# MinJunKang/DualPixelFace

Measured on AMD Instinct MI355X. Metric: train samples/sec, StereoDPNet 1024x1536 DP pair, higher is better.
Workload: dtype f32

## Files before the change

dualpixelface_amd/csrc/conv_igemm2.hip:

```cpp
#include "conv_internal.h"
#include <cstdlib>
#include <type_traits>

namespace {

constexpr int MAXT = 27;
constexpr int NLD = 8;
constexpr int ZPAGE = 16;

struct G2P {
  int N, C, K, Ktot, k0;
  int ID, IH, IW, OD, OH, OW;
  int sxd, sxh, sxw;
  int e0d, e0h, e0w;
  int ext_d, ext_h;
  int pz, thp, thp_shift, odt;
  int planeStride;
  int RS, SR;
  int colshift;
  int rpc, chanStride;
  int nseg;
  int nwseg;
  int T;
  int tilesH, tilesW;
// ... 914 lines not shown
    } else {
      wpk[base] = (unsigned short)(sh & 0xffffu);
      wpk[base + 512LL * MT] = (unsigned short)(sm & 0xffffu);
      wpk[base + 1024LL * MT] = (unsigned short)(sl & 0xffffu);
    }
  }
}

struct T2P {
  int N, C, K, Ktot, k0;
  int ID, IH, IW, OD, OH, OW;
  int RS, SR, rpc, chanStride, nseg, nwseg, nchunks;
  int tilesH, tilesW, ntiles, cpx, QD;
  unsigned mSR, mRPC, mEH;
  int vec;
};

struct T2Combo { int cls, tap; };
struct T2Unit { int e, n; T2Combo c[8]; };
struct T2Table { T2Unit u[8]; };

constexpr T2Table t2_table() {
  T2Table tb{};
  const int order[8] = {0, 1, 2, 3, 5, 6, 7, 4};
  for (int ui = 0; ui < 8; ++ui) {
    const int e = order[ui];
    const int es[3] = {e >> 2, (e >> 1) & 1, e & 1};
    T2Unit& u = tb.u[ui];
    u.e = e;
    u.n = 0;
// ... 200 lines not shown
      const int od = 2 * qd + rd, oh = 2 * qh + rh, ow = 2 * qw;
      if (od >= p.OD || oh >= p.OH || ow >= p.OW) continue;
      float* op = on + ((long long)od * p.OH + oh) * p.OW + ow;
      if (quad_ok) {
        const bool odd = (l31 & 1) != 0;
#pragma unroll
        for (int j = 0; j < 16; j += 2) {
          const float a0 = acc[rd * 4 + rh * 2][j], a1 = acc[rd * 4 + rh * 2 + 1][j];
          const float b0 = acc[rd * 4 + rh * 2][j + 1], b1 = acc[rd * 4 + rh * 2 + 1][j + 1];
          const float s0 = odd ? a0 : b0, s1 = odd ? a1 : b1;
          const float t0 = __builtin_bit_cast(float, __builtin_amdgcn_mov_dpp(__builtin_bit_cast(int, s0), 0xB1, 0xf, 0xf, true));
          const float t1 = __builtin_bit_cast(float, __builtin_amdgcn_mov_dpp(__builtin_bit_cast(int, s1), 0xB1, 0xf, 0xf, true));
          const int k = ((j + (odd ? 1 : 0)) & 3) + 8 * (j >> 2) + 4 * hh;
          if (k < p.K) {
            const float bv = bias ? bias[p.k0 + k] : 0.f;
            const f32x4 v = odd ? f32x4{t0 + bv, t1 + bv, b0 + bv, b1 + bv} : f32x4{a0 + bv, a1 + bv, t0 + bv, t1 + bv};
            *reinterpret_cast<f32x4*>(on + ((long long)od * p.OH + oh) * p.OW + (ow & ~3) + (long long)k * kstride) = v;
          }
        }
        continue;
      }
#pragma unroll
      for (int j = 0; j < 16; ++j) {
        const int k = (j & 3) + 8 * (j >> 2) + 4 * hh;
        if (k < p.K) {
          const float bv = bias ? bias[p.k0 + k] : 0.f;
          const float v0 = acc[rd * 4 + rh * 2][j] + bv, v1 = acc[rd * 4 + rh * 2 + 1][j] + bv;
          float* o = op + (long long)k * kstride;
          if (pair_ok) {
            *reinterpret_cast<float2*>(o) = make_float2(v0, v1);
          } else {
            o[0] = v0;
            if (ow + 1 < p.OW) o[1] = v1;
          }
        }
      }
    }
}

__global__ void igemm2_pack_kernel(const float* __restrict__ w, float* __restrict__ wpk, int wA, int wB, int T, int KT, int CC, int nchunks,
                                   int mode, int k0, int K, int C) {
  const long long total = (long long)nchunks * T * CC * KT + ZPAGE;
  for (long long i = (long long)blockIdx.x * blockDim.x + threadIdx.x; i < total; i += (long long)gridDim.x * blockDim.x) {
    float v = 0.f;
    if (i >= ZPAGE) {
      const long long e = i - ZPAGE;
      const int k = (int)(e % KT);
      const int cc = (int)((e / KT) % CC);
// ... 184 lines not shown
  p.N = d.N; p.C = d.C; p.Ktot = d.Ktot;
  p.ID = d.ID; p.IH = d.IH; p.IW = d.IW; p.OD = d.OD; p.OH = d.OH; p.OW = d.OW;
  p.RS = 36; p.SR = 9; p.rpc = 2 * 5; p.chanStride = p.rpc * p.RS;
  p.nseg = CC * p.rpc * p.SR;
  p.nwseg = bf ? 27 * 32 : 27 * CC * 32 / 4;
  p.nchunks = (d.C + CC - 1) / CC;
  p.QD = dpf_div_up(d.OD, 2);
  p.tilesH = dpf_div_up(dpf_div_up(d.OH, 2), 4);
  p.tilesW = dpf_div_up(dpf_div_up(d.OW, 2), 32);
  const long long ntiles = (long long)d.N * p.QD * p.tilesH * p.tilesW;
  if (ntiles <= 0 || ntiles > 0x3fffffffLL) return DPF_ERR_INVALID_ARG;
  p.ntiles = (int)ntiles;
  p.cpx = (int)((ntiles + 7) / 8);
  p.mSR = magic20(p.SR); p.mRPC = magic20(p.rpc); p.mEH = magic20(5);
  p.vec = env_int("DPF_G2_VEC_STORE", 1);
  const size_t lds = 2 * (size_t)(CC * p.chanStride + 4 * p.nwseg) * sizeof(float);
  for (int k0 = 0; k0 < d.K; k0 += 32) {
    const int Kc = d.K - k0 < 32 ? d.K - k0 : 32;
    p.K = Kc; p.k0 = d.k0 + k0;
    const long long total = (long long)p.nchunks * 27 * CC * 32 + ZPAGE;
    if (bf)
      hipLaunchKernelGGL(igemm2_pack_bf16_kernel, dim3(dpf_ew_grid(total)), dim3(256), 0, st, w, reinterpret_cast<unsigned short*>(ws), d.wA, d.wB, 27,
                         32, p.nchunks, d.mode, p.k0, Kc, d.C);
    else
      hipLaunchKernelGGL(igemm2_pack_kernel, dim3(dpf_ew_grid(total)), dim3(256), 0, st, w, ws, d.wA, d.wB, 27, 32, CC, p.nchunks, d.mode, p.k0, Kc, d.C);
    if (dpf_check_launch() != DPF_OK) return DPF_ERR_LAUNCH;
    int rc;
    if (bf) {
      rc = launch_t2<8, true>(x, ws, bias, out, p, lds, st);
      if (rc != DPF_OK) return rc;
// ... 14 lines not shown
  const long long x9 = (g4 > g8 ? g4 : g8) * 3 * (KT / 32) * 256;
  return plain > x9 ? plain : x9;
}

int dpf_igemm2_conv(const float* x, const float* w, const float* bias, float* out, float* ws, const DpfConvDesc& d, hipStream_t st,
                    DpfConvStats* stats) {
  static const int enabled = env_int("DPF_IGEMM2", 1);
  if (!enabled) return DPF_ERR_UNSUPPORTED;
  const int T = d.kd * d.kh * d.kw;
  if (T > MAXT || d.K > 128) return DPF_ERR_UNSUPPORTED;
  if ((d.IW & 3) || (reinterpret_cast<uintptr_t>(x) & 15) || (reinterpret_cast<uintptr_t>(ws) & 15)) return DPF_ERR_UNSUPPORTED;
  const long long x_chan = (long long)d.ID * d.IH * d.IW;
  if (9 * x_chan >= (1LL << 30)) return DPF_ERR_UNSUPPORTED;
  if (T == 1 && !env_int("DPF_IGEMM2_1x1", 1)) return DPF_ERR_UNSUPPORTED;
  if (stats && (d.transposed || d.Ktot != d.K)) return DPF_ERR_UNSUPPORTED;
  if (d.accumulate && d.transposed && (d.sd != 1 || d.sh != 1 || d.sw != 1)) return DPF_ERR_UNSUPPORTED;
  if (d.transposed && (d.sd != 1 || d.sh != 1 || d.sw != 1)) return igemm2_tr2(x, w, bias, out, ws, d, st);

  const int MT = (d.K + 31) / 32, KT = 32 * MT;
  static const int nt_over = 0, cc_over = 0, lds_target = 53 * 1024;
  int NT = MT == 1 ? 4 : 2;
  if (nt_over == 2 || (nt_over == 4 && MT <= 2)) NT = nt_over;
  bool bf = dpf_conv_operand_bf16() != 0 && T > 1;
  const bool bf_mode = bf;
  static const int bf3_on = env_int("DPF_IGEMM3_BF", 1);
  int p_single = 0;
  if (bf) {
    auto patch_for = [&](int nt) {
      const int sxh = d.transposed ? 1 : d.sh, sxw = d.transposed ? 1 : d.sw;
      const int e0w = d.transposed ? d.pw - (d.kw - 1) * d.dw : -d.pw;
      const int ext_d = (d.kd - 1) * d.dd + 1, ext_h = (4 * nt - 1) * sxh + (d.kh - 1) * d.dh + 1, ext_w = 31 * sxw + (d.kw - 1) * d.dw + 1;
// ... 184 lines not shown
```

dualpixelface_amd/csrc/norm_act.hip:

```cpp
#include "dpf_common.h"

namespace {

constexpr int ROW_CHUNK = 4096;

template <bool DET> struct RedAcc { typedef float type; };
template <> struct RedAcc<true> { typedef double type; };

__device__ __forceinline__ float red_block_sum(float v, float* sm4) { return dpf_block_sum_256(v, sm4); }
__device__ __forceinline__ float red_block_sum(double v, float* sm4) {
#pragma unroll
  for (int o = 32; o > 0; o >>= 1) v += __shfl_xor(v, o, 64);
  double* smd = reinterpret_cast<double*>(sm4);
  const int w = threadIdx.x >> 6;
  __syncthreads();
  if ((threadIdx.x & 63) == 0) smd[w] = v;
  __syncthreads();
  return (float)((smd[0] + smd[1]) + (smd[2] + smd[3]));
}

template <bool DET>
__global__ __launch_bounds__(256) void bn_stats_kernel(const float* __restrict__ x, float* __restrict__ sums, int N, int C, long long S,
                                                       int chunk) {
  __shared__ float sm[8];
// ... 273 lines not shown
  if (ACT == DPF_ACT_PRELU) {
    const float slf = red_block_sum(sl, sm);
    if (threadIdx.x == 0) atomicAdd(&sums[3 * c + 2], slf);
  }
}

template <int ACT, bool RES>
__global__ __launch_bounds__(256) void bn_bwd_apply_kernel(const float* __restrict__ x, const float* __restrict__ dy,
                                                           const float* __restrict__ mean, const float* __restrict__ invstd,
                                                           const float* __restrict__ w, const float* __restrict__ bsh, int wmod,
                                                           const float* __restrict__ res, int act, const float* __restrict__ slope_p,
                                                           float slope_c, const float* __restrict__ sums, float inv_count,
                                                           int training, float* __restrict__ dx, float* __restrict__ dres, int C,
                                                           long long S, const float* __restrict__ count_dev, int gC = 0, int gc0 = 0,
                                                           float* __restrict__ fin_dweight = nullptr, float* __restrict__ fin_dbias = nullptr,
                                                           float* __restrict__ fin_dslope = nullptr) {
  const int row = blockIdx.y;
  if (blockIdx.x == 0 && blockIdx.y == 0 && (fin_dweight || fin_dbias || fin_dslope)) {
    for (int cp = threadIdx.x; cp < wmod; cp += 256) {
      float a = 0.f, b = 0.f;
      for (int c = cp; c < C; c += wmod) {
        a += sums[3 * c];
        b += sums[3 * c + 1];
      }
      if (fin_dbias) fin_dbias[cp] = a;
      if (fin_dweight) fin_dweight[cp] = b;
    }
    if (fin_dslope && threadIdx.x == 0) {
      float sl = 0.f;
      for (int c = 0; c < C; ++c) sl += sums[3 * c + 2];
      fin_dslope[0] = sl;
// ... 23 lines not shown
    const float z = fmaf(xh, g, be) + rv;
    o_dz = d * dact_t<ACT>(z, slope);
    o_dx = mean ? gi * (o_dz - m_dz - xh * m_dzx) : o_dz;
  };
  (void)act;
  if ((S & 3) == 0) {
#pragma unroll 2
    for (long long s = s0 + 4 * threadIdx.x; s < s1; s += 4 * 256) {
      const v4f xv = ld4(x + base + s);
      const v4f dv = ld4(dy + base + s);
      v4f rv = {0.f, 0.f, 0.f, 0.f};
      if (RES) rv = ld4(res + base + s);
      float z0, z1, z2, z3, x0, x1, x2, x3;
      one(xv.x, rv.x, dv.x, z0, x0); one(xv.y, rv.y, dv.y, z1, x1);
      one(xv.z, rv.z, dv.z, z2, x2); one(xv.w, rv.w, dv.w, z3, x3);
      if (dres) *reinterpret_cast<v4f*>(dres + base + s) = v4f{z0, z1, z2, z3};
      if (dx) *reinterpret_cast<v4f*>(dx + base + s) = v4f{x0, x1, x2, x3};
    }
  } else {
    for (long long s = s0 + threadIdx.x; s < s1; s += 256) {
      float oz, ox;
      one(x[base + s], RES ? res[base + s] : 0.f, dy[base + s], oz, ox);
      if (dres) dres[base + s] = oz;
      if (dx) dx[base + s] = ox;
    }
  }
}

__global__ void bn_bwd_finalize_kernel(const float* __restrict__ sums, int C, int wmod, float* __restrict__ dweight,
                                       float* __restrict__ dbias, float* __restrict__ dslope) {
  const int cp = blockIdx.x * blockDim.x + threadIdx.x;
  if (cp < wmod) {
    float a = 0.f, b = 0.f;
    for (int c = cp; c < C; c += wmod) {
      a += sums[3 * c];
      b += sums[3 * c + 1];
    }
    if (dbias) dbias[cp] = a;
    if (dweight) dweight[cp] = b;
// ... 117 lines not shown
int dpf_norm_act_forward_slice(const float* x, const float* mean, const float* invstd, const float* w, const float* b, int wmod,
                               const float* res, const float* res2, int act, const float* slope, float slope_const, float* y, int y_channels,
                               int y_c0, int N, int C, long long S, void* stream) {
  dpf_clear_error();
  if (!x || !y || N <= 0 || C <= 0 || S <= 0 || (long long)N * C > 65535 || y_c0 < 0 || y_c0 + C > y_channels) return DPF_ERR_INVALID_ARG;
  if (wmod <= 0) wmod = C;
#define DPF_CALL(A, R) hipLaunchKernelGGL((bn_apply_kernel<A, R>), row_grid(N * C, S), dim3(256), 0, (hipStream_t)stream, x, mean, invstd, w, b, wmod, res, res2, act, slope, slope_const, y, C, S, y_channels, y_c0)
  DPF_ACT_DISPATCH(act, (res != nullptr || res2 != nullptr), DPF_CALL)
#undef DPF_CALL
  return dpf_check_launch();
}

static int norm_act_backward_impl(const float* x, const float* dy, int gC, int gc0, const float* mean, const float* invstd, const float* w,
                                  const float* b, int wmod, const float* res, int act, const float* slope, float slope_const, int training,
                                  float* dx, float* dres, float* dweight, float* dbias, float* dslope, float* ws, int N, int C, long long S,
                                  int phase, double count, void* stream) {
  dpf_clear_error();
  if (!x || !dy || !ws || N <= 0 || C <= 0 || S <= 0 || (long long)N * C > 65535 || phase < 0 || phase > 3) return DPF_ERR_INVALID_ARG;
  if (wmod <= 0) wmod = C;
  hipStream_t st = (hipStream_t)stream;
  const bool need_reduce = (mean != nullptr) || (act == DPF_ACT_PRELU && dslope);
  bool fused_fin = false;
  if (need_reduce && phase != 2) {
    if (phase != 3 && hipMemsetAsync(ws, 0, sizeof(float) * 3 * C, st) != hipSuccess) return DPF_ERR_LAUNCH;
    const int chunk = reduce_chunk(N * C, S);
    const bool det = dpf_deterministic() != 0;
#define DPF_CALL(A, R)                                                                                                                              \
  do {                                                                                                                                              \
    if (det) hipLaunchKernelGGL((bn_bwd_reduce_kernel<A, R, true>), dim3(1, (unsigned)C), dim3(256), 0, st, x, dy, mean, invstd, w, b, wmod, res, \
                                act, slope, slope_const, ws, N, C, S, chunk, gC, gc0);                                                             \
    else hipLaunchKernelGGL((bn_bwd_reduce_kernel<A, R, false>), reduce_grid(N * C, S, chunk), dim3(256), 0, st, x, dy, mean, invstd, w, b, wmod,   \
// ... 1 lines not shown
  } while (0)
    DPF_ACT_DISPATCH(act, (res != nullptr), DPF_CALL)
#undef DPF_CALL
    fused_fin = (dx || dres) && phase != 1;
    if (!fused_fin)
      hipLaunchKernelGGL(bn_bwd_finalize_kernel, dim3(dpf_div_up(wmod, 64)), dim3(64), 0, st, ws, C, wmod, mean ? dweight : nullptr,
                         mean ? dbias : nullptr, act == DPF_ACT_PRELU ? dslope : nullptr);
  }
  if ((dx || dres) && phase != 1) {
    const float* count_dev = (phase == 2 && count < 0) ? ws + 3 * (long long)C : nullptr;
    if (count <= 0) count = (double)N * (double)S;
    const float inv_cnt = (float)(1.0 / count);
    float* fdw = (fused_fin && mean) ? dweight : nullptr;
    float* fdb = (fused_fin && mean) ? dbias : nullptr;
    float* fds = (fused_fin && act == DPF_ACT_PRELU) ? dslope : nullptr;
#define DPF_CALL(A, R) hipLaunchKernelGGL((bn_bwd_apply_kernel<A, R>), row_grid(N * C, S), dim3(256), 0, st, x, dy, mean, invstd, w, b, wmod, res, act, slope, slope_const, ws, inv_cnt, training, dx, dres, C, S, count_dev, gC, gc0, fdw, fdb, fds)
    DPF_ACT_DISPATCH(act, (res != nullptr), DPF_CALL)
#undef DPF_CALL
  }
  return dpf_check_launch();
}

int dpf_norm_act_backward_ex(const float* x, const float* dy, const float* mean, const float* invstd, const float* w, const float* b,
                             int wmod, const float* res, int act, const float* slope, float slope_const, int training, float* dx,
                             float* dres, float* dweight, float* dbias, float* dslope, float* ws, int N, int C, long long S, int phase,
                             double count, void* stream) {
  return norm_act_backward_impl(x, dy, 0, 0, mean, invstd, w, b, wmod, res, act, slope, slope_const, training, dx, dres, dweight, dbias,
                                dslope, ws, N, C, S, phase, count, stream);
}

int dpf_norm_act_backward_slice(const float* x, const float* dy, int dy_channels, int dy_c0, const float* mean, const float* invstd,
                                const float* w, const float* b, int wmod, const float* res, int act, const float* slope, float slope_const,
                                int training, float* dx, float* dres, float* dweight, float* dbias, float* dslope, float* ws, int N, int C,
                                long long S, void* stream) {
  if (dy_c0 < 0 || dy_c0 + C > dy_channels) return DPF_ERR_INVALID_ARG;
  return norm_act_backward_impl(x, dy, dy_channels, dy_c0, mean, invstd, w, b, wmod, res, act, slope, slope_const, training, dx, dres,
                                dweight, dbias, dslope, ws, N, C, S, 0, 0.0, stream);
}

int dpf_norm_act_backward_slice_ex(const float* x, const float* dy, int dy_channels, int dy_c0, const float* mean, const float* invstd,
                                   const float* w, const float* b, int wmod, const float* res, int act, const float* slope, float slope_const,
                                   int training, float* dx, float* dres, float* dweight, float* dbias, float* dslope, float* ws, int N, int C,
                                   long long S, int phase, double count, void* stream) {
// ... 23 lines not shown
```

dualpixelface_amd/ops.py:

```python
import ctypes
import os

import torch

from ._lib import lib, DpfError, ERRORS

ACT_NONE, ACT_RELU, ACT_PRELU, ACT_LEAKY, ACT_SIGMOID = 0, 1, 2, 3, 4
BN_EPS, BN_MOMENTUM = 1e-5, 0.1
FUSE_BN_STATS = os.environ.get('DPF_FUSE_BN_STATS', '1') != '0'

_scratch = {}

PROFILE = None
PROFILE_DETAIL = False


class _Timed(object):
    def __init__(self, family, flops, tag='', nbytes=0.0):
        self.family, self.flops, self.tag, self.nbytes = family, flops, tag, nbytes

    def __enter__(self):
        if PROFILE is not None:
            self.e0 = torch.cuda.Event(enable_timing=True)
            self.e1 = torch.cuda.Event(enable_timing=True)
# ... 186 lines not shown
    ws = _conv_ws((kd, kh, kw), C, K, x.device)
    with _dense_timed('fwd', x, K, (kd, kh, kw), stride, dil, od * oh * ow, x.numel() + out.numel() + w.numel()):
        if stats is not None and FUSE_BN_STATS and K <= 128 and IW % 4 == 0 and kd * kh * kw > 1:
            cap = int(L.call('dpf_conv_stats_slab_doubles', N, K, od, oh, ow))
            slab = torch.empty(cap, dtype=torch.float64, device=x.device)
            parts = ctypes.c_int(0)
            if _supported('dpf_conv_forward_stats', _ptr(x), _ptr(w), _ptr(bias), _ptr(out), _ptr(ws), N, C, ID, IH, IW, K, kd, kh, kw,
                          *stride, *pad, *dil, _ptr(slab), cap, ctypes.byref(parts), _stream()):
                stats.update(slab=slab, parts=int(parts.value), count=N * od * oh * ow, channels=K, ptr=out.data_ptr())
                return out
        L.call('dpf_conv_forward', _ptr(x), _ptr(w), _ptr(bias), _ptr(out), _ptr(ws), N, C, ID, IH, IW, K, kd, kh, kw,
               *stride, *pad, *dil, _stream())
    return out


def _conv_transpose_raw(x, w, bias, out_dims, ksize, stride, pad, dil, k_needed=None):
    N, C, ID, IH, IW = x.shape
    K = w.shape[1]
    kd, kh, kw = ksize
    out = torch.empty((N, K) + tuple(out_dims), dtype=torch.float32, device=x.device)
    L = lib()
    if (C <= 4 and bias is None and k_needed is None and tuple(stride) == (1, 1, 1) and tuple(dil) == (1, 1, 1) and kh == 3 and kw == 3
            and out_dims[2] % 4 == 0):
        with _Timed('conv_smallk', 2.0 * N * K * C * kd * kh * kw * ID * IH * IW, 'skd N%d C%d K%d in%dx%dx%d' % (N, C, K, ID, IH, IW)):
            done = _supported('dpf_conv_smallk_dgrad', _ptr(x), _ptr(w), _ptr(out), N, K, *out_dims, C, kd, kh, kw, *pad, _stream())
        if done:
            return out
    if k_needed is not None and 0 < k_needed < K:
        out[:, k_needed:].zero_()
        entry, chans = 'dpf_conv_transpose_ex', (k_needed, K)
    else:
        entry, chans = 'dpf_conv_transpose', (K,)
    ws = _conv_ws(ksize, C, K, x.device)
    with _dense_timed('tr ', x, chans[0], ksize, stride, dil, ID * IH * IW, x.numel() + out.numel() * chans[0] // K + w.numel()):
        L.call(entry, _ptr(x), _ptr(w), _ptr(bias), _ptr(out), _ptr(ws), N, C, ID, IH, IW, *chans, *out_dims, kd, kh, kw,
# ... 76 lines not shown
        gw = _conv_wgrad_raw(g, x, wshape, stride, pad, dil)
    g.record_stream(side)
    x.record_stream(side)
    _wgrad_pending.append((p, gw.view(p.shape)))
    return None


def _channel_sum(g):
    N, C = g.shape[0], g.shape[1]
    S = g.numel() // (N * C)
    out = torch.zeros(C, dtype=torch.float32, device=g.device)
    lib().call('dpf_channel_sum', _ptr(g), _ptr(out), N, C, S, _stream())
    return out


class ConvFn(torch.autograd.Function):

    @staticmethod
    def forward(ctx, x, w, bias, stride, pad, dil, gi_channels=None, stats=None):
        x, w = _c(x), _c(w)
        _need(x, w, bias)
        ctx.cfg = (stride, pad, dil)
        ctx.gi_channels = gi_channels
        ctx.save_for_backward(x, w)
        ctx.has_bias = bias is not None
        ctx.bf16 = CONV_OPERANDS_BF16
        return _conv_fwd_raw(x, w, bias, stride, pad, dil, stats)

    @staticmethod
    def backward(ctx, gy):
        x, w = ctx.saved_tensors
        stride, pad, dil = ctx.cfg
        gy = _c(gy)
        gx = gw = gb = None
        with conv_operands(ctx.bf16):
            if ctx.needs_input_grad[0]:
                gx = _conv_transpose_raw(gy, w, None, x.shape[2:], w.shape[2:], stride, pad, dil, k_needed=ctx.gi_channels)
            if ctx.needs_input_grad[1]:
                gw = _wgrad_dispatch(w, gy, x, w.shape, stride, pad, dil)
        if ctx.has_bias and ctx.needs_input_grad[2]:
            gb = _channel_sum(gy)
        return gx, gw, gb, None, None, None, None, None


class ConvTransposeFn(torch.autograd.Function):

    @staticmethod
    def forward(ctx, x, w, stride, pad, outpad):
        x, w = _c(x), _c(w)
        _need(x, w)
        ks = tuple(w.shape[2:])
        dil = (1, 1, 1)
        out_dims = tuple((x.shape[2 + i] - 1) * stride[i] - 2 * pad[i] + ks[i] + outpad[i] for i in range(3))
        ctx.cfg = (stride, pad, dil)
        ctx.save_for_backward(x, w)
        ctx.bf16 = CONV_OPERANDS_BF16
        return _conv_transpose_raw(x, w, None, out_dims, ks, stride, pad, dil)
# ... 1 lines not shown
    @staticmethod
    def backward(ctx, gy):
        x, w = ctx.saved_tensors
        stride, pad, dil = ctx.cfg
        gy = _c(gy)
        gx = gw = None
        with conv_operands(ctx.bf16):
            if ctx.needs_input_grad[0]:
                gx = _conv_fwd_raw(gy, w, None, stride, pad, dil)
            if ctx.needs_input_grad[1]:
                gw = _wgrad_dispatch(w, x, gy, w.shape, stride, pad, dil)
        return gx, gw, None, None, None


def conv3d(x, w, bias=None, stride=1, pad=0, dil=1, gi_channels=None, stats=None):
    return ConvFn.apply(x, w, bias, _t3(stride), _t3(pad), _t3(dil), gi_channels, stats)


class ConvBf16Fn(torch.autograd.Function):

    @staticmethod
    def forward(ctx, x, w, bias, stride, pad, dil):
        x, w = _c(x), _c(w)
        _need(x, w, bias)
        N, C, IH, IW = x.shape
        K, kh, kw = w.shape[0], w.shape[2], w.shape[3]
        oh, ow = _out_dim(IH, kh, stride, pad, dil), _out_dim(IW, kw, stride, pad, dil)
        out = torch.empty((N, K, oh, ow), dtype=torch.float32, device=x.device)
        L = lib()
        ws = scratch((L.call('dpf_conv2d_bf16_workspace_bytes', C, K, kh * kw) + 3) // 4, x.device, 'convw')
        with _Timed('conv_bf16', 2.0 * N * K * C * kh * kw * oh * ow, 'b16 N%d C%d K%d in%dx%d k%d%d s%d d%d' % (N, C, K, IH, IW, kh, kw, stride, dil)):
# ... 20 lines not shown
                ws = scratch((L.call('dpf_conv2d_bf16_workspace_bytes', C, K, kh * kw) + 3) // 4, x.device, 'convw')
                with _Timed('conv_bf16', 2.0 * N * K * C * kh * kw * IH * IW, 'b16t N%d C%d K%d in%dx%d k%d%d d%d' % (N, K, C, IH, IW, kh, kw, dil)):
                    L.call('dpf_conv2d_bf16_dgrad', _ptr(gy), _ptr(w), _ptr(gx), _ptr(ws), N, C, IH, IW, K, kh, kw, pad, pad, dil, dil, _stream())
            else:
                gx = _conv_transpose_raw(gy.unsqueeze(2), w.unsqueeze(2), None, (1, IH, IW), (1, kh, kw), s3, p3, d3).squeeze(2)
        if ctx.needs_input_grad[1]:
            gw = _conv_wgrad_raw(gy.unsqueeze(2), x.unsqueeze(2), (K, C, 1, kh, kw), s3, p3, d3).squeeze(2)
        if ctx.has_bias and ctx.needs_input_grad[2]:
            gb = _channel_sum(gy)
        return gx, gw, gb, None, None, None


def conv2d(x, w, bias=None, stride=1, pad=0, dil=1, bf16=False, stats=None):
    if bf16 and w.shape[0] > 4:
        return ConvBf16Fn.apply(x, w, bias, int(stride), int(pad), int(dil))
    y = ConvFn.apply(x.unsqueeze(2), w.unsqueeze(2), bias, (1, stride, stride), (0, pad, pad), (1, dil, dil), None, stats)
    return y.squeeze(2)


def conv_transpose3d(x, w, stride=2, pad=1, outpad=1):
    return ConvTransposeFn.apply(x, w, _t3(stride), _t3(pad), _t3(outpad))


def conv_transpose2d(x, w, stride=2, pad=1):
    s, q = int(stride), int(pad)
    return ConvTransposeFn.apply(x.unsqueeze(2), w.unsqueeze(2), (1, s, s), (0, q, q), (0, 0, 0)).squeeze(2)


class DepthwiseGeneralFn(torch.autograd.Function):

    @staticmethod
# ... 124 lines not shown
               _ptr(running_var), _ptr(mean), _ptr(invstd), _stream())
        holder.clear()
        read_x = False
    else:
        momentum, rm, rv = (BN_MOMENTUM, running_mean, running_var) if mode == 1 else (0.0, None, None)
        L.call('dpf_bn_stats', _ptr(x), N, C, S, BN_EPS, momentum, _ptr(rm), _ptr(rv), _ptr(mean), _ptr(invstd),
               _ptr(scratch(2 * C, x.device)), _stream())
    if mode == 1:
        _bn_order_after(running_mean)
    return mean, invstd, read_x


class NormActFn(torch.autograd.Function):

    @staticmethod
    def forward(ctx, x, weight, bias, slope, res, res2, running_mean, running_var, mode, act, slope_const, exchange=None, stats=None):
        x = _c(x)
        res = None if res is None else _c(res)
        res2 = None if res2 is None else _c(res2)
        _need(x, weight, bias, slope, res, res2)
        N, C = x.shape[0], x.shape[1]
        S = x.numel() // (N * C)
        L = lib()
        n_, c_ = (1, N * C) if mode == 3 else (N, C)
        wmod = C
        sync = exchange if mode == 1 else None
        with _detail('naf') as timer:
            moments = _bn_sync_gather([x], sync)[0] if sync is not None else None
            mean, invstd, read_x = _bn_stats(x, mode, running_mean, running_var, stats, moments)
            timer.nbytes = 4.0 * x.numel() * (read_x + 2 + (res is not None) + (res2 is not None))
            y = torch.empty_like(x)
            L.call('dpf_norm_act_forward', _ptr(x), _ptr(mean), _ptr(invstd), _ptr(weight), _ptr(bias), wmod, _ptr(res), _ptr(res2), act,
                   _ptr(slope), float(slope_const), _ptr(y), n_, c_, S, _stream())
        ctx.save_for_backward(x, weight, bias, slope, res, mean, invstd)
        ctx.cfg = (mode, act, float(slope_const), n_, c_, S, wmod, res2 is not None)
        ctx.exchange = sync
        return y

    @staticmethod
    def backward(ctx, gy):
        x, weight, bias, slope, res, mean, invstd = ctx.saved_tensors
        mode, act, slope_const, n_, c_, S, wmod, has_res2 = ctx.cfg
        gy = _c(gy)
        L = lib()
        need_dx = ctx.needs_input_grad[0]
        dx = torch.empty_like(x) if need_dx else None
        dres = torch.empty_like(x) if (res is not None and ctx.needs_input_grad[4]) else None
        dweight = torch.empty_like(weight) if (weight is not None and ctx.needs_input_grad[1]) else None
        dbias = torch.empty_like(bias) if (bias is not None and ctx.needs_input_grad[2]) else None
        dslope = torch.empty_like(slope) if (slope is not None and ctx.needs_input_grad[3]) else None
        training = 1 if mode in (1, 3) else 0
        args = (_ptr(x), _ptr(gy), _ptr(mean), _ptr(invstd), _ptr(weight), _ptr(bias), wmod, _ptr(res), act, _ptr(slope), slope_const,
                training, _ptr(dx), _ptr(dres), _ptr(dweight), _ptr(dbias), _ptr(dslope))
        with _detail('nab', 4.0 * x.numel() * ((2 if training else 0) + 2 + (dx is not None) + (dres is not None))):
            if ctx.exchange is not None:
                ws = torch.empty(3 * c_ + 1, dtype=torch.float32, device=x.device)
                L.call('dpf_norm_act_backward_ex', *args, _ptr(ws), n_, c_, S, 1, 0.0, _stream())
                ws[3 * c_:].fill_(float(n_) * float(S))
                ctx.exchange.all_reduce_sum_(ws)
                L.call('dpf_norm_act_backward_ex', *args, _ptr(ws), n_, c_, S, 2, -1.0, _stream())
            else:
                ws = zero_slot(3 * c_, x.device)
                L.call('dpf_norm_act_backward_ex', *args, _ptr(ws), n_, c_, S, 3, 0.0, _stream())
        dres2 = gy if (has_res2 and ctx.needs_input_grad[5]) else None
        return dx, dweight, dbias, dslope, dres, dres2, None, None, None, None, None, None, None


def norm_act(x, weight=None, bias=None, slope=None, res=None, res2=None, running_mean=None, running_var=None, mode=0, act=ACT_NONE,
             slope_const=0.0, exchange=None, stats=None):
    return NormActFn.apply(x, weight, bias, slope, res, res2, running_mean, running_var, mode, act, slope_const, exchange, stats)


class NormActCatFn(torch.autograd.Function):

    @staticmethod
    def forward(ctx, mode, act, holders, exchange, *tensors):
        n = len(tensors) // 5
        xs = [_c(tensors[5 * i]) for i in range(n)]
        ws = [tensors[5 * i + 1] for i in range(n)]
        bs = [tensors[5 * i + 2] for i in range(n)]
        rms = [tensors[5 * i + 3] for i in range(n)]
        rvs = [tensors[5 * i + 4] for i in range(n)]
        _need(*xs)
        N = xs[0].shape[0]
        Cs = [x.shape[1] for x in xs]
# ... 801 lines not shown
```

dualpixelface_amd/stereodpnet.py:

```python
import math
import os

import torch

from . import ops
from .core import ArenaModule, Spec, cost_levels, set_levels
from .ops import ACT_NONE, ACT_RELU, ACT_PRELU, ACT_LEAKY, ACT_SIGMOID
from .sampler_tables import build_phase_tables, build_shift_tables, is_fractional


def _dpblock_spec(s, p, c, t):
    for n in ('conv1', 'conv2'):
        s.convbn2(p + '.%s.0' % n, c, c)
        s.prelu(p + '.%s.1' % n)
    for i in range(3):
        s.convbn2(p + '.conv_dilate.%d' % i, c, c)
    s.convbn2(p + '.conv3', 3 * c, c)
    s.convbn2(p + '.conv4.0', c, t * c)
    s.prelu(p + '.conv4.1')
    s.conv(p + '.conv5.depthwise', t * c, 1, (3, 3))
    s.conv(p + '.conv5.pointwise', t * c, t * c, (1, 1))
    s.bn(p + '.conv5.bn', t * c)
    s.prelu(p + '.conv5.prelu')
    s.conv(p + '.conv_skip', t * c, c, (1, 1), bias=('uniform', 1.0 / math.sqrt(c)))
# ... 17 lines not shown
        ag = 'aggregation'
        s.convbn3(ag + '.dres0.0', cin, c)
        s.convbn3(ag + '.dres0.2', c, c)
        s.convbn3(ag + '.dres1.0', c, c)
        s.convbn3(ag + '.dres1.2', c, c)
        for n in ('dres2', 'dres3', 'dres4'):
            hourglass(ag + '.' + n)
        for n in ('classif1', 'classif2', 'classif3'):
            s.convbn3(ag + '.%s.0' % n, c, c)
            s.conv(ag + '.%s.2' % n, 1, c, (3, 3, 3))

    def _hourglass(self, x, p, presqu, postsqu):
        P = self._P
        out = self._convbn3(x, p + '.conv1.0', 2, ACT_RELU)
        pre = self._convbn3(out, p + '.conv2', 1, ACT_RELU, postsqu)
        out = self._convbn3(pre, p + '.conv3.0', 2, ACT_RELU)
        out = self._convbn3(out, p + '.conv4.0', 1, ACT_RELU)
        up = ops.conv_transpose3d(out, P[p + '.conv5.0.weight'])
        post = self._bn(up, p + '.conv5.1', ACT_RELU, None, presqu if presqu is not None else pre)
        up = ops.conv_transpose3d(post, P[p + '.conv6.0.weight'])
        return up, pre, post

    def _aggregate(self, cost):
        P, p = self._P, 'aggregation'
        c0 = self._convbn3(cost, p + '.dres0.0', 1, ACT_RELU)
        c0 = self._convbn3(c0, p + '.dres0.2', 1, ACT_RELU)
        r = self._convbn3(c0, p + '.dres1.0', 1, ACT_RELU)
        c0 = self._convbn3(r, p + '.dres1.2', 1, ACT_NONE, c0)
        u1, pre1, post1 = self._hourglass(c0, p + '.dres2', None, None)
        o1 = self._bn(u1, p + '.dres2.conv6.1', ACT_NONE, None, c0)
        u2, _, post2 = self._hourglass(o1, p + '.dres3', pre1, post1)
        o2 = self._bn(u2, p + '.dres3.conv6.1', ACT_NONE, None, c0)
        u3, _, _ = self._hourglass(o2, p + '.dres4', pre1, post2)
        o3 = self._bn(u3, p + '.dres4.conv6.1', ACT_NONE, None, c0)

        def head(x, q):
            y = self._convbn3(x, q + '.0', 1, ACT_RELU)
            return ops.conv3d(y, P[q + '.2.weight'], None, 1, 1, 1)

        k1 = head(o1, p + '.classif1')
        k2 = ops.norm_act(head(o2, p + '.classif2'), res=k1)
        k3 = ops.norm_act(head(o3, p + '.classif3'), res=k2)
        if self.training:
            return [k3, k2, k1], [o3, o2, o1]
        return [k3], [o3]


# ... 95 lines not shown
            for q, d in zip(prefixes, dilations):
                y = ops.conv2d(x, P[q + '.0.weight'], None, 1, d if d > 1 else 1, d, bf16=self.bf16_2d)
                if self.training:
                    self._count(q + '.1.num_batches_tracked')
                branches.append((y, P[q + '.1.weight'], P[q + '.1.bias'], B[q + '.1.running_mean'], B[q + '.1.running_var'], None))
            return ops.norm_act_concat(branches, 1 if self.training else 2, ACT_NONE, exchange=sync)
        branches = []
        for q in prefixes:
            if self.training:
                self._count(q + '.1.num_batches_tracked')
            branches.append((P[q + '.0.weight'], P[q + '.1.weight'], P[q + '.1.bias'], B[q + '.1.running_mean'], B[q + '.1.running_var']))
        return ops.conv_bn_concat(x, branches, [d if d > 1 else 1 for d in dilations], self.training)

    def _dpblock(self, x, p, s):
        P = self._P
        o1 = self._convbn2(x, p + '.conv1.0', act=ACT_PRELU, slope=P[p + '.conv1.1.weight'])
        o2 = self._convbn2(o1, p + '.conv2.0', act=ACT_PRELU, slope=P[p + '.conv2.1.weight'])
        o2 = self._convbn2_concat(o2, [p + '.conv_dilate.%d' % i for i in range(3)], [2 * i + 1 for i in range(3)])
        o = self._convbn2(o2, p + '.conv3', act=ACT_PRELU, slope=P[p + '.prelu.weight'], res=o1)
        o = self._convbn2(o, p + '.conv4.0', s, s, 2, act=ACT_PRELU, slope=P[p + '.conv4.1.weight'])
        d = ops.depthwise_conv3x3(o, P[p + '.conv5.depthwise.weight'])
        d = self._conv2d(d, P[p + '.conv5.pointwise.weight'])
        skip = self._conv2d(x, P[p + '.conv_skip.weight'], P[p + '.conv_skip.bias'], s)
        return self._bn(d, p + '.conv5.bn', ACT_PRELU, P[p + '.conv5.prelu.weight'], None, skip)

    def _features(self, img):
        P, p = self._P, 'feature_extraction'
        x = self._convbn2(img, p + '.firstconv.0', 2, 1, 1, ACT_RELU)
        x = self._convbn2(x, p + '.firstconv.2', act=ACT_RELU)
        x = self._convbn2(x, p + '.firstconv.4', act=ACT_RELU)
        o1 = self._dpblock(x, p + '.block1', 2)
        o2 = o1
# ... 151 lines not shown
```

include/dpf_hip.h:

```cpp
#ifndef DPF_HIP_H
#define DPF_HIP_H

#ifdef __cplusplus
extern "C" {
#endif

#define DPF_OK 0
#define DPF_ERR_INVALID_ARG (-1)
#define DPF_ERR_LAUNCH (-2)
#define DPF_ERR_UNSUPPORTED (-3)

#define DPF_ACT_NONE 0
#define DPF_ACT_RELU 1
#define DPF_ACT_PRELU 2
#define DPF_ACT_LEAKY 3
#define DPF_ACT_SIGMOID 4

long long dpf_conv_workspace_floats(int T, int reduce, int outc);
int dpf_conv_forward(const float* x, const float* w, const float* bias, float* out, float* ws, int N, int C, int ID, int IH, int IW,
                     int K, int kd, int kh, int kw, int sd, int sh, int sw, int pd, int ph, int pw, int dd, int dh, int dw,
                     void* stream);
int dpf_conv_transpose(const float* x, const float* w, const float* bias, float* out, float* ws, int N, int C, int ID, int IH, int IW,
                       int K, int OD, int OH, int OW, int kd, int kh, int kw, int sd, int sh, int sw, int pd, int ph, int pw,
                       int dd, int dh, int dw, void* stream);
// ... 53 lines not shown
                          float* dres, float* dweight, float* dbias, float* dslope, float* ws, int N, int C, long long S, void* stream);
int dpf_norm_act_forward_slice(const float* x, const float* mean, const float* invstd, const float* w, const float* b, int wmod,
                               const float* res, const float* res2, int act, const float* slope, float slope_const, float* y, int y_channels,
                               int y_c0, int N, int C, long long S, void* stream);
int dpf_norm_act_backward_slice(const float* x, const float* dy, int dy_channels, int dy_c0, const float* mean, const float* invstd,
                                const float* w, const float* b, int wmod, const float* res, int act, const float* slope, float slope_const,
                                int training, float* dx, float* dres, float* dweight, float* dbias, float* dslope, float* ws, int N, int C,
                                long long S, void* stream);
int dpf_bn_local_moments(const float* x, int N, int C, long long S, float* moments, float* ws, void* stream);
int dpf_bn_merge_moments(const float* moments, const float* counts, int W, int C, float eps, float momentum, float* running_mean,
                         float* running_var, float* mean, float* invstd, void* stream);
int dpf_norm_act_backward_ex(const float* x, const float* dy, const float* mean, const float* invstd, const float* w, const float* b,
                             int wmod, const float* res, int act, const float* slope, float slope_const, int training, float* dx,
                             float* dres, float* dweight, float* dbias, float* dslope, float* ws, int N, int C, long long S, int phase,
                             double count, void* stream);
int dpf_norm_act_backward_slice_ex(const float* x, const float* dy, int dy_channels, int dy_c0, const float* mean, const float* invstd,
                                   const float* w, const float* b, int wmod, const float* res, int act, const float* slope, float slope_const,
                                   int training, float* dx, float* dres, float* dweight, float* dbias, float* dslope, float* ws, int N, int C,
                                   long long S, int phase, double count, void* stream);
int dpf_channel_sum(const float* g, float* out, int N, int C, long long S, void* stream);

int dpf_upsample_bilinear2d_forward(const float* x, float* y, long long NC, int h, int w, int H, int W, void* stream);
int dpf_upsample_bilinear2d_backward(const float* g, float* dx, long long NC, int h, int w, int H, int W, void* stream);
int dpf_resize_bilinear2d_forward(const float* x, float* y, long long NC, int h, int w, int H, int W, int align_corners, void* stream);
int dpf_resize_bilinear2d_backward(const float* g, float* dx, long long NC, int h, int w, int H, int W, int align_corners, void* stream);
int dpf_upsample_nearest_add_forward(const float* lat, const float* top, float* y, long long NC, int h, int w, int H, int W, void* stream);
int dpf_upsample_nearest_backward(const float* g, float* dtop, long long NC, int h, int w, int H, int W, void* stream);

int dpf_shift_triple_forward(const float* fea, float* out, const int* iy, const float* wy, const int* ix, const float* wx, int B, int C,
                             int h, int w, void* stream);
// ... 106 lines not shown
```

Measured before the change: 26.84.

## Accumulate fan-out gradients in place via shared sink buffers

Adds a gradient sink for tensors consumed by several ops, so each consumer's backward (conv input-grad, norm-act residual grad) writes or accumulates straight into one shared buffer instead of autograd summing separate gradient tensors. The igemm2 transposed-conv epilogue and the BN backward apply kernel gain read-modify-write accumulate modes, and the model marks the fan-out points. The aim is to cut allocations and extra elementwise add passes in backward. It adds a read of the destination on accumulate, cross-stream ordering logic, and relies on autograd calling the consumers' backwards before the fan-out node.

```diff
diff --git a/dualpixelface_amd/csrc/conv_igemm2.hip b/dualpixelface_amd/csrc/conv_igemm2.hip
--- a/dualpixelface_amd/csrc/conv_igemm2.hip
+++ b/dualpixelface_amd/csrc/conv_igemm2.hip
@@ -952,6 +952,7 @@
   int tilesH, tilesW, ntiles, cpx, QD;
   unsigned mSR, mRPC, mEH;
   int vec;
+  int accum;
 };
 
 struct T2Combo { int cls, tap; };
@@ -1182,8 +1183,10 @@
           const int k = ((j + (odd ? 1 : 0)) & 3) + 8 * (j >> 2) + 4 * hh;
           if (k < p.K) {
             const float bv = bias ? bias[p.k0 + k] : 0.f;
-            const f32x4 v = odd ? f32x4{t0 + bv, t1 + bv, b0 + bv, b1 + bv} : f32x4{a0 + bv, a1 + bv, t0 + bv, t1 + bv};
-            *reinterpret_cast<f32x4*>(on + ((long long)od * p.OH + oh) * p.OW + (ow & ~3) + (long long)k * kstride) = v;
+            f32x4 v = odd ? f32x4{t0 + bv, t1 + bv, b0 + bv, b1 + bv} : f32x4{a0 + bv, a1 + bv, t0 + bv, t1 + bv};
+            f32x4* o = reinterpret_cast<f32x4*>(on + ((long long)od * p.OH + oh) * p.OW + (ow & ~3) + (long long)k * kstride);
+            if (p.accum) v += *o;
+            *o = v;
           }
         }
         continue;
@@ -1193,13 +1196,18 @@
         const int k = (j & 3) + 8 * (j >> 2) + 4 * hh;
         if (k < p.K) {
           const float bv = bias ? bias[p.k0 + k] : 0.f;
-          const float v0 = acc[rd * 4 + rh * 2][j] + bv, v1 = acc[rd * 4 + rh * 2 + 1][j] + bv;
+          float v0 = acc[rd * 4 + rh * 2][j] + bv, v1 = acc[rd * 4 + rh * 2 + 1][j] + bv;
           float* o = op + (long long)k * kstride;
           if (pair_ok) {
+            if (p.accum) {
+              const float2 old = *reinterpret_cast<const float2*>(o);
+              v0 += old.x;
+              v1 += old.y;
+            }
             *reinterpret_cast<float2*>(o) = make_float2(v0, v1);
           } else {
-            o[0] = v0;
-            if (ow + 1 < p.OW) o[1] = v1;
+            o[0] = p.accum ? o[0] + v0 : v0;
+            if (ow + 1 < p.OW) o[1] = p.accum ? o[1] + v1 : v1;
           }
         }
       }
@@ -1414,6 +1422,7 @@
   p.cpx = (int)((ntiles + 7) / 8);
   p.mSR = magic20(p.SR); p.mRPC = magic20(p.rpc); p.mEH = magic20(5);
   p.vec = env_int("DPF_G2_VEC_STORE", 1);
+  p.accum = d.accumulate;
   const size_t lds = 2 * (size_t)(CC * p.chanStride + 4 * p.nwseg) * sizeof(float);
   for (int k0 = 0; k0 < d.K; k0 += 32) {
     const int Kc = d.K - k0 < 32 ? d.K - k0 : 32;
@@ -1458,7 +1467,6 @@
   if (9 * x_chan >= (1LL << 30)) return DPF_ERR_UNSUPPORTED;
   if (T == 1 && !env_int("DPF_IGEMM2_1x1", 1)) return DPF_ERR_UNSUPPORTED;
   if (stats && (d.transposed || d.Ktot != d.K)) return DPF_ERR_UNSUPPORTED;
-  if (d.accumulate && d.transposed && (d.sd != 1 || d.sh != 1 || d.sw != 1)) return DPF_ERR_UNSUPPORTED;
   if (d.transposed && (d.sd != 1 || d.sh != 1 || d.sw != 1)) return igemm2_tr2(x, w, bias, out, ws, d, st);
 
   const int MT = (d.K + 31) / 32, KT = 32 * MT;
diff --git a/dualpixelface_amd/csrc/norm_act.hip b/dualpixelface_amd/csrc/norm_act.hip
--- a/dualpixelface_amd/csrc/norm_act.hip
+++ b/dualpixelface_amd/csrc/norm_act.hip
@@ -311,7 +311,8 @@
                                                            int training, float* __restrict__ dx, float* __restrict__ dres, int C,
                                                            long long S, const float* __restrict__ count_dev, int gC = 0, int gc0 = 0,
                                                            float* __restrict__ fin_dweight = nullptr, float* __restrict__ fin_dbias = nullptr,
-                                                           float* __restrict__ fin_dslope = nullptr) {
+                                                           float* __restrict__ fin_dslope = nullptr, int accum = 0) {
+  const bool acc_dx = (accum & 1) != 0, acc_dres = (accum & 2) != 0;
   const int row = blockIdx.y;
   if (blockIdx.x == 0 && blockIdx.y == 0 && (fin_dweight || fin_dbias || fin_dslope)) {
     for (int cp = threadIdx.x; cp < wmod; cp += 256) {
@@ -365,15 +366,29 @@
       float z0, z1, z2, z3, x0, x1, x2, x3;
       one(xv.x, rv.x, dv.x, z0, x0); one(xv.y, rv.y, dv.y, z1, x1);
       one(xv.z, rv.z, dv.z, z2, x2); one(xv.w, rv.w, dv.w, z3, x3);
-      if (dres) *reinterpret_cast<v4f*>(dres + base + s) = v4f{z0, z1, z2, z3};
-      if (dx) *reinterpret_cast<v4f*>(dx + base + s) = v4f{x0, x1, x2, x3};
+      if (dres) {
+        v4f* o = reinterpret_cast<v4f*>(dres + base + s);
+        if (acc_dres) {
+          const v4f old = *o;
+          z0 = __fadd_rn(old.x, z0); z1 = __fadd_rn(old.y, z1); z2 = __fadd_rn(old.z, z2); z3 = __fadd_rn(old.w, z3);
+        }
+        *o = v4f{z0, z1, z2, z3};
+      }
+      if (dx) {
+        v4f* o = reinterpret_cast<v4f*>(dx + base + s);
+        if (acc_dx) {
+          const v4f old = *o;
+          x0 = __fadd_rn(old.x, x0); x1 = __fadd_rn(old.y, x1); x2 = __fadd_rn(old.z, x2); x3 = __fadd_rn(old.w, x3);
+        }
+        *o = v4f{x0, x1, x2, x3};
+      }
     }
   } else {
     for (long long s = s0 + threadIdx.x; s < s1; s += 256) {
       float oz, ox;
       one(x[base + s], RES ? res[base + s] : 0.f, dy[base + s], oz, ox);
-      if (dres) dres[base + s] = oz;
-      if (dx) dx[base + s] = ox;
+      if (dres) dres[base + s] = acc_dres ? __fadd_rn(dres[base + s], oz) : oz;
+      if (dx) dx[base + s] = acc_dx ? __fadd_rn(dx[base + s], ox) : ox;
     }
   }
 }
@@ -521,7 +536,7 @@
 static int norm_act_backward_impl(const float* x, const float* dy, int gC, int gc0, const float* mean, const float* invstd, const float* w,
                                   const float* b, int wmod, const float* res, int act, const float* slope, float slope_const, int training,
                                   float* dx, float* dres, float* dweight, float* dbias, float* dslope, float* ws, int N, int C, long long S,
-                                  int phase, double count, void* stream) {
+                                  int phase, double count, void* stream, int accum = 0) {
   dpf_clear_error();
   if (!x || !dy || !ws || N <= 0 || C <= 0 || S <= 0 || (long long)N * C > 65535 || phase < 0 || phase > 3) return DPF_ERR_INVALID_ARG;
   if (wmod <= 0) wmod = C;
@@ -553,7 +568,7 @@
     float* fdw = (fused_fin && mean) ? dweight : nullptr;
     float* fdb = (fused_fin && mean) ? dbias : nullptr;
     float* fds = (fused_fin && act == DPF_ACT_PRELU) ? dslope : nullptr;
-#define DPF_CALL(A, R) hipLaunchKernelGGL((bn_bwd_apply_kernel<A, R>), row_grid(N * C, S), dim3(256), 0, st, x, dy, mean, invstd, w, b, wmod, res, act, slope, slope_const, ws, inv_cnt, training, dx, dres, C, S, count_dev, gC, gc0, fdw, fdb, fds)
+#define DPF_CALL(A, R) hipLaunchKernelGGL((bn_bwd_apply_kernel<A, R>), row_grid(N * C, S), dim3(256), 0, st, x, dy, mean, invstd, w, b, wmod, res, act, slope, slope_const, ws, inv_cnt, training, dx, dres, C, S, count_dev, gC, gc0, fdw, fdb, fds, accum)
     DPF_ACT_DISPATCH(act, (res != nullptr), DPF_CALL)
 #undef DPF_CALL
   }
@@ -566,6 +581,15 @@
                              double count, void* stream) {
   return norm_act_backward_impl(x, dy, 0, 0, mean, invstd, w, b, wmod, res, act, slope, slope_const, training, dx, dres, dweight, dbias,
                                 dslope, ws, N, C, S, phase, count, stream);
+}
+
+int dpf_norm_act_backward_acc(const float* x, const float* dy, const float* mean, const float* invstd, const float* w, const float* b,
+                              int wmod, const float* res, int act, const float* slope, float slope_const, int training, float* dx,
+                              float* dres, float* dweight, float* dbias, float* dslope, float* ws, int N, int C, long long S, int phase,
+                              double count, int acc_dx, int acc_dres, void* stream) {
+  if (dx && dx == dres) return DPF_ERR_INVALID_ARG;
+  return norm_act_backward_impl(x, dy, 0, 0, mean, invstd, w, b, wmod, res, act, slope, slope_const, training, dx, dres, dweight, dbias,
+                                dslope, ws, N, C, S, phase, count, stream, (acc_dx ? 1 : 0) | (acc_dres ? 2 : 0));
 }
 
 int dpf_norm_act_backward_slice(const float* x, const float* dy, int dy_channels, int dy_c0, const float* mean, const float* invstd,
diff --git a/dualpixelface_amd/ops.py b/dualpixelface_amd/ops.py
--- a/dualpixelface_amd/ops.py
+++ b/dualpixelface_amd/ops.py
@@ -224,11 +224,12 @@
     return out
 
 
-def _conv_transpose_raw(x, w, bias, out_dims, ksize, stride, pad, dil, k_needed=None):
+def _conv_transpose_raw(x, w, bias, out_dims, ksize, stride, pad, dil, k_needed=None, out=None):
     N, C, ID, IH, IW = x.shape
     K = w.shape[1]
     kd, kh, kw = ksize
-    out = torch.empty((N, K) + tuple(out_dims), dtype=torch.float32, device=x.device)
+    if out is None:
+        out = torch.empty((N, K) + tuple(out_dims), dtype=torch.float32, device=x.device)
     L = lib()
     if (C <= 4 and bias is None and k_needed is None and tuple(stride) == (1, 1, 1) and tuple(dil) == (1, 1, 1) and kh == 3 and kw == 3
             and out_dims[2] % 4 == 0):
@@ -335,14 +336,81 @@
     return out
 
 
+class GradSink(object):
+
+    def __init__(self, like):
+        self.shape, self.device = tuple(like.shape), like.device
+        self.buf = None
+        self.stream = None
+
+    def _order(self):
+        cur = torch.cuda.current_stream(self.device)
+        if self.stream is not None and self.stream.cuda_stream != cur.cuda_stream:
+            cur.wait_stream(self.stream)
+            self.buf.record_stream(cur)
+        self.stream = cur
+
+    def target(self, shape=None):
+        acc = 0 if self.buf is None else 1
+        if self.buf is None:
+            self.buf = torch.empty(self.shape, dtype=torch.float32, device=self.device)
+        self._order()
+        return (self.buf if shape is None else self.buf.view(shape)), acc
+
+    def add(self, g):
+        g = _c(g)
+        N, C = self.shape[0], self.shape[1]
+        buf, acc = self.target()
+        lib().call('dpf_copy_channels', _ptr(g), _ptr(buf), N, C, 0, C, 0, C, g.numel() // (N * C), acc, _stream())
+
+    def take(self):
+        buf = self.buf
+        if buf is not None:
+            self._order()
+        self.buf = self.stream = None
+        return buf
+
+
+class FanOutFn(torch.autograd.Function):
+
+    @staticmethod
+    def forward(ctx, x, sink):
+        ctx.sink = sink
+        ctx.set_materialize_grads(False)
+        return x.view_as(x)
+
+    @staticmethod
+    def backward(ctx, g):
+        sink = ctx.sink
+        if sink.buf is None:
+            return g, None
+        if g is not None:
+            sink.add(g)
+        return sink.take(), None
+
+
+def fan_out(x):
+    if not (torch.is_grad_enabled() and x.requires_grad):
+        return x
+    sink = GradSink(x)
+    y = FanOutFn.apply(x, sink)
+    y._dpf_sink = sink
+    return y
+
+
+def _sink_of(t):
+    return getattr(t, '_dpf_sink', None) if t is not None else None
+
+
 class ConvFn(torch.autograd.Function):
 
     @staticmethod
-    def forward(ctx, x, w, bias, stride, pad, dil, gi_channels=None, stats=None):
+    def forward(ctx, x, w, bias, stride, pad, dil, gi_channels=None, stats=None, sink=None):
         x, w = _c(x), _c(w)
         _need(x, w, bias)
         ctx.cfg = (stride, pad, dil)
         ctx.gi_channels = gi_channels
+        ctx.sink = sink if gi_channels is None else None
         ctx.save_for_backward(x, w)
         ctx.has_bias = bias is not None
         ctx.bf16 = CONV_OPERANDS_BF16
@@ -355,13 +423,19 @@
         gy = _c(gy)
         gx = gw = gb = None
         with conv_operands(ctx.bf16):
-            if ctx.needs_input_grad[0]:
+            if ctx.needs_input_grad[0] and ctx.sink is not None:
+                dst, acc = ctx.sink.target(x.shape)
+                if acc:
+                    _conv_transpose_acc(gy, w, dst, w.shape[2:], stride, pad, dil)
+                else:
+                    _conv_transpose_raw(gy, w, None, x.shape[2:], w.shape[2:], stride, pad, dil, out=dst)
+            elif ctx.needs_input_grad[0]:
                 gx = _conv_transpose_raw(gy, w, None, x.shape[2:], w.shape[2:], stride, pad, dil, k_needed=ctx.gi_channels)
             if ctx.needs_input_grad[1]:
                 gw = _wgrad_dispatch(w, gy, x, w.shape, stride, pad, dil)
         if ctx.has_bias and ctx.needs_input_grad[2]:
             gb = _channel_sum(gy)
-        return gx, gw, gb, None, None, None, None, None
+        return gx, gw, gb, None, None, None, None, None, None
 
 
 class ConvTransposeFn(torch.autograd.Function):
@@ -393,7 +467,7 @@
 
 
 def conv3d(x, w, bias=None, stride=1, pad=0, dil=1, gi_channels=None, stats=None):
-    return ConvFn.apply(x, w, bias, _t3(stride), _t3(pad), _t3(dil), gi_channels, stats)
+    return ConvFn.apply(x, w, bias, _t3(stride), _t3(pad), _t3(dil), gi_channels, stats, _sink_of(x))
 
 
 class ConvBf16Fn(torch.autograd.Function):
@@ -444,7 +518,7 @@
 def conv2d(x, w, bias=None, stride=1, pad=0, dil=1, bf16=False, stats=None):
     if bf16 and w.shape[0] > 4:
         return ConvBf16Fn.apply(x, w, bias, int(stride), int(pad), int(dil))
-    y = ConvFn.apply(x.unsqueeze(2), w.unsqueeze(2), bias, (1, stride, stride), (0, pad, pad), (1, dil, dil), None, stats)
+    y = ConvFn.apply(x.unsqueeze(2), w.unsqueeze(2), bias, (1, stride, stride), (0, pad, pad), (1, dil, dil), None, stats, _sink_of(x))
     return y.squeeze(2)
 
 
@@ -599,7 +673,8 @@
 class NormActFn(torch.autograd.Function):
 
     @staticmethod
-    def forward(ctx, x, weight, bias, slope, res, res2, running_mean, running_var, mode, act, slope_const, exchange=None, stats=None):
+    def forward(ctx, x, weight, bias, slope, res, res2, running_mean, running_var, mode, act, slope_const, exchange=None, stats=None,
+                res_sink=None):
         x = _c(x)
         res = None if res is None else _c(res)
         res2 = None if res2 is None else _c(res2)
@@ -620,6 +695,7 @@
         ctx.save_for_backward(x, weight, bias, slope, res, mean, invstd)
         ctx.cfg = (mode, act, float(slope_const), n_, c_, S, wmod, res2 is not None)
         ctx.exchange = sync
+        ctx.res_sink = res_sink if res is not None else None
         return y
 
     @staticmethod
@@ -630,30 +706,33 @@
         L = lib()
         need_dx = ctx.needs_input_grad[0]
         dx = torch.empty_like(x) if need_dx else None
-        dres = torch.empty_like(x) if (res is not None and ctx.needs_input_grad[4]) else None
+        dres = torch.empty_like(x) if (res is not None and ctx.needs_input_grad[4] and ctx.res_sink is None) else None
+        dres_dst, dres_acc = (dres, 0) if (ctx.res_sink is None or not ctx.needs_input_grad[4]) else ctx.res_sink.target(x.shape)
         dweight = torch.empty_like(weight) if (weight is not None and ctx.needs_input_grad[1]) else None
         dbias = torch.empty_like(bias) if (bias is not None and ctx.needs_input_grad[2]) else None
         dslope = torch.empty_like(slope) if (slope is not None and ctx.needs_input_grad[3]) else None
         training = 1 if mode in (1, 3) else 0
         args = (_ptr(x), _ptr(gy), _ptr(mean), _ptr(invstd), _ptr(weight), _ptr(bias), wmod, _ptr(res), act, _ptr(slope), slope_const,
-                training, _ptr(dx), _ptr(dres), _ptr(dweight), _ptr(dbias), _ptr(dslope))
-        with _detail('nab', 4.0 * x.numel() * ((2 if training else 0) + 2 + (dx is not None) + (dres is not None))):
+                training, _ptr(dx), _ptr(dres_dst), _ptr(dweight), _ptr(dbias), _ptr(dslope))
+        tail = (0, dres_acc, _stream())
+        with _detail('nab', 4.0 * x.numel() * ((2 if training else 0) + 2 + (dx is not None) + (dres_dst is not None) + dres_acc)):
             if ctx.exchange is not None:
                 ws = torch.empty(3 * c_ + 1, dtype=torch.float32, device=x.device)
                 L.call('dpf_norm_act_backward_ex', *args, _ptr(ws), n_, c_, S, 1, 0.0, _stream())
                 ws[3 * c_:].fill_(float(n_) * float(S))
                 ctx.exchange.all_reduce_sum_(ws)
-                L.call('dpf_norm_act_backward_ex', *args, _ptr(ws), n_, c_, S, 2, -1.0, _stream())
+                L.call('dpf_norm_act_backward_acc', *args, _ptr(ws), n_, c_, S, 2, -1.0, *tail)
             else:
                 ws = zero_slot(3 * c_, x.device)
-                L.call('dpf_norm_act_backward_ex', *args, _ptr(ws), n_, c_, S, 3, 0.0, _stream())
+                L.call('dpf_norm_act_backward_acc', *args, _ptr(ws), n_, c_, S, 3, 0.0, *tail)
         dres2 = gy if (has_res2 and ctx.needs_input_grad[5]) else None
-        return dx, dweight, dbias, dslope, dres, dres2, None, None, None, None, None, None, None
+        return dx, dweight, dbias, dslope, dres, dres2, None, None, None, None, None, None, None, None
 
 
 def norm_act(x, weight=None, bias=None, slope=None, res=None, res2=None, running_mean=None, running_var=None, mode=0, act=ACT_NONE,
              slope_const=0.0, exchange=None, stats=None):
-    return NormActFn.apply(x, weight, bias, slope, res, res2, running_mean, running_var, mode, act, slope_const, exchange, stats)
+    return NormActFn.apply(x, weight, bias, slope, res, res2, running_mean, running_var, mode, act, slope_const, exchange, stats,
+                           _sink_of(res))
 
 
 class NormActCatFn(torch.autograd.Function):
diff --git a/dualpixelface_amd/stereodpnet.py b/dualpixelface_amd/stereodpnet.py
--- a/dualpixelface_amd/stereodpnet.py
+++ b/dualpixelface_amd/stereodpnet.py
@@ -55,6 +55,8 @@
         P = self._P
         out = self._convbn3(x, p + '.conv1.0', 2, ACT_RELU)
         pre = self._convbn3(out, p + '.conv2', 1, ACT_RELU, postsqu)
+        if presqu is None:
+            pre = ops.fan_out(pre)
         out = self._convbn3(pre, p + '.conv3.0', 2, ACT_RELU)
         out = self._convbn3(out, p + '.conv4.0', 1, ACT_RELU)
         up = ops.conv_transpose3d(out, P[p + '.conv5.0.weight'])
@@ -65,13 +67,13 @@
     def _aggregate(self, cost):
         P, p = self._P, 'aggregation'
         c0 = self._convbn3(cost, p + '.dres0.0', 1, ACT_RELU)
-        c0 = self._convbn3(c0, p + '.dres0.2', 1, ACT_RELU)
+        c0 = ops.fan_out(self._convbn3(c0, p + '.dres0.2', 1, ACT_RELU))
         r = self._convbn3(c0, p + '.dres1.0', 1, ACT_RELU)
-        c0 = self._convbn3(r, p + '.dres1.2', 1, ACT_NONE, c0)
+        c0 = ops.fan_out(self._convbn3(r, p + '.dres1.2', 1, ACT_NONE, c0))
         u1, pre1, post1 = self._hourglass(c0, p + '.dres2', None, None)
-        o1 = self._bn(u1, p + '.dres2.conv6.1', ACT_NONE, None, c0)
+        o1 = ops.fan_out(self._bn(u1, p + '.dres2.conv6.1', ACT_NONE, None, c0))
         u2, _, post2 = self._hourglass(o1, p + '.dres3', pre1, post1)
-        o2 = self._bn(u2, p + '.dres3.conv6.1', ACT_NONE, None, c0)
+        o2 = ops.fan_out(self._bn(u2, p + '.dres3.conv6.1', ACT_NONE, None, c0))
         u3, _, _ = self._hourglass(o2, p + '.dres4', pre1, post2)
         o3 = self._bn(u3, p + '.dres4.conv6.1', ACT_NONE, None, c0)
 
@@ -197,8 +199,9 @@
 
     def _dpblock(self, x, p, s):
         P = self._P
-        o1 = self._convbn2(x, p + '.conv1.0', act=ACT_PRELU, slope=P[p + '.conv1.1.weight'])
-        o2 = self._convbn2(o1, p + '.conv2.0', act=ACT_PRELU, slope=P[p + '.conv2.1.weight'])
+        x = ops.fan_out(x)
+        o1 = ops.fan_out(self._convbn2(x, p + '.conv1.0', act=ACT_PRELU, slope=P[p + '.conv1.1.weight']))
+        o2 = ops.fan_out(self._convbn2(o1, p + '.conv2.0', act=ACT_PRELU, slope=P[p + '.conv2.1.weight']))
         o2 = self._convbn2_concat(o2, [p + '.conv_dilate.%d' % i for i in range(3)], [2 * i + 1 for i in range(3)])
         o = self._convbn2(o2, p + '.conv3', act=ACT_PRELU, slope=P[p + '.prelu.weight'], res=o1)
         o = self._convbn2(o, p + '.conv4.0', s, s, 2, act=ACT_PRELU, slope=P[p + '.conv4.1.weight'])
diff --git a/include/dpf_hip.h b/include/dpf_hip.h
--- a/include/dpf_hip.h
+++ b/include/dpf_hip.h
@@ -91,6 +91,10 @@
                              int wmod, const float* res, int act, const float* slope, float slope_const, int training, float* dx,
                              float* dres, float* dweight, float* dbias, float* dslope, float* ws, int N, int C, long long S, int phase,
                              double count, void* stream);
+int dpf_norm_act_backward_acc(const float* x, const float* dy, const float* mean, const float* invstd, const float* w, const float* b,
+                              int wmod, const float* res, int act, const float* slope, float slope_const, int training, float* dx,
+                              float* dres, float* dweight, float* dbias, float* dslope, float* ws, int N, int C, long long S, int phase,
+                              double count, int acc_dx, int acc_dres, void* stream);
 int dpf_norm_act_backward_slice_ex(const float* x, const float* dy, int dy_channels, int dy_c0, const float* mean, const float* invstd,
                                    const float* w, const float* b, int wmod, const float* res, int act, const float* slope, float slope_const,
                                    int training, float* dx, float* dres, float* dweight, float* dbias, float* dslope, float* ws, int N, int C,
```

Result: no change. 27.05, median of 6 (+0.8%).
